# balazs-bamer/cuda-bezier-triangle-raytracer

Measured on AMD Instinct MI355X. Metric: Mrays/sec (primary+refracted) at 1/2/4/8 MI355X; % of HBM-read roofline, higher is better.
Workload: dtype f32; 1 GPU; cfg4: two stacked cfg2 lenses at x=10 and x=13, 4096x4096 rays; image=4096x4096, primaries_per_gpu=16777216, patches=6144, parallelism=64x64 image tiles round-robin over 1 rank(s), strong scaling, pipeline=fused, frames_in_flight=3, scan=BVH-culled (bit-identical to brute force), numerics=parity: bit-identical to the CPU oracle

## Files before the change

cuda-bezier-triangle-raytracer_amd/bzr_amd/__init__.py:

```python
from __future__ import annotations

import ctypes
import os
from contextlib import contextmanager
from pathlib import Path

import numpy as np

PKG_DIR = Path(__file__).resolve().parent.parent
LIB_PATH = Path(os.environ.get("BZR_LIBRARY", PKG_DIR / "lib" / "libbzr.so"))

OK = 0
HOST_PTRS, DEVICE_PTRS = 0, 1
MODE_PARITY, MODE_FAST = 0, 2
ACCEL_NONE = 4
PIPELINE_STAGED = 8
PIPELINE_FUSED = 16
RAYS_AOS = 32
WHAT_FOLLOW0, WHAT_FOLLOW1, WHAT_FOLLOW2, WHAT_NONE, WHAT_INTERSECT = 0, 1, 2, 3, 4
LIMIT_THIS, LIMIT_NONE = 0, 1
RR_NONE, RR_INSIDE, RR_OUTSIDE = 0, 1, 2
ENVELOPE_ELLIPSOID, ENVELOPE_TESTLENS = 0, 1
PATCH_WORDS = 66
KERNELS = ("k_traverse", "bucket", "k_newton", "k_follow", "k_finish", "k_overflow", "k_intersect_scan",
           "k_refract_scan", "k_chain_scan", "k_patch", "k_newton_lane", "k_trace")
COUNTERS = ("segments", "pairs", "follows", "overflow_rays", "lane_chunks", "node_visits", "leaf_fetches",
            "gate_tests", "newton_rounds", "rounds_odd", "runs_odd", "dirty_rows")
HIT_FIELDS = 13

_P = ctypes.c_void_p
_U32 = ctypes.c_uint32
_I32 = ctypes.c_int32
_F = ctypes.c_float

_SIGS = {
    "bzr_abi_version": [],
    "bzr_last_error": [],
    "bzr_device_count": [ctypes.POINTER(_I32)],
    "bzr_ctx_create": [_I32, ctypes.POINTER(_P)],
    "bzr_ctx_destroy": [_P],
    "bzr_ctx_set_stream": [_P, _P],
    "bzr_ctx_use_own_stream": [_P],
# ... 616 lines not shown
```

cuda-bezier-triangle-raytracer_amd/csrc/device/patch_math.hpp:

```cpp
#pragma once
#include <hip/hip_runtime.h>
#include <cfloat>
#include <cstdint>

namespace bzr_dev {

struct f3 {
  float x, y, z;
};
__device__ __forceinline__ f3 mk(float x, float y, float z) { return f3{x, y, z}; }
namespace rec {
constexpr int kUnder = 0;
constexpr int kDivider = 4;
constexpr int kNeigh = 16;
constexpr int kCp = 19;
constexpr int kMinv = 49;
constexpr int kHin = 58;
constexpr int kHout = 59;
constexpr int kDirA = 60;
constexpr int kDirB = 63;
constexpr int kWords = 66;
}

struct Patch {
// ... 153 lines not shown
__device__ __forceinline__ f3 unit_or_self(f3 a, float z) {
  if (!(z > 0.0f)) return a;
  float r = __builtin_amdgcn_rsqf(z);
  return mk(a.x * r, a.y * r, a.z * r);
}
__device__ __forceinline__ void div_heights(float hin, float hout, float ic, float &din, float &dout) {
  din = div_rn(hin, ic);
  dout = div_rn(hout, ic);
}
#include "patch_math_body.inc"
#pragma clang fp contract(off)
}

using namespace exact;

template <bool kGated = false, bool kFast = false, typename P>
__device__ __forceinline__ Hit patch_intersect(const P &p, f3 s, f3 d, bool limitNone) {
  Hit h;
  h.t = 0.0f;
  h.point = mk(0.0f, 0.0f, 0.0f);
  h.cs = 0.0f;
  h.bary = h.point;
  h.normal = h.point;
  h.what = kNone;
  f3 ip;
  float ic, it;
  bool valid = plane_ray(p.n(), p.c(), s, d, ip, ic, it);
  (void)valid;
#if BZR_PASS_FLAT
  if (!kGated) {
    const f3 b0 = matvec(p, ip);
    const bool in = (b0.x >= 0.0f) & (b0.x <= 1.0f) & (b0.y >= 0.0f) & (b0.y <= 1.0f) & (b0.z >= 0.0f) & (b0.z <= 1.0f);
    const bool ok = valid & (fabsf(it) > -p.hin()) & (fabsf(it) > p.hout()) & (limitNone | in);
    Hit r;
    if constexpr (kFast) r = fast::newton_tail(p, s, d, ic, it);
    else r = newton_tail(p, s, d, ic, it);
    return ok ? r : h;
  }
#endif
  if (!kGated) {
    if (!(valid && fabsf(it) > -p.hin() && fabsf(it) > p.hout())) return h;
    f3 b0 = matvec(p, ip);
    if (!(limitNone || (b0.x >= 0.0f && b0.x <= 1.0f && b0.y >= 0.0f && b0.y <= 1.0f && b0.z >= 0.0f && b0.z <= 1.0f)))
      return h;
  }
  if constexpr (kFast) return fast::newton_tail(p, s, d, ic, it);
  else return newton_tail(p, s, d, ic, it);
}

}
```

cuda-bezier-triangle-raytracer_amd/csrc/device/patch_math_body.inc:

```
__device__ __forceinline__ f3 add(f3 a, f3 b) { return mk(a.x + b.x, a.y + b.y, a.z + b.z); }
__device__ __forceinline__ f3 sub(f3 a, f3 b) { return mk(a.x - b.x, a.y - b.y, a.z - b.z); }
__device__ __forceinline__ f3 scale(f3 a, float s) { return mk(a.x * s, a.y * s, a.z * s); }
__device__ __forceinline__ float dot(f3 a, f3 b) { return a.x * b.x + (a.y * b.y + a.z * b.z); }
__device__ __forceinline__ f3 cross(f3 a, f3 b) {
  return mk(a.y * b.z - a.z * b.y, a.z * b.x - a.x * b.z, a.x * b.y - a.y * b.x);
}
__device__ __forceinline__ f3 normalized(f3 a) {
  float z = dot(a, a);
  return unit_or_self(a, z);
}

template <typename P>
__device__ __forceinline__ f3 matvec(const P &p, f3 v) {
  return mk(p.m(0) * v.x + (p.m(3) * v.y + p.m(6) * v.z), p.m(1) * v.x + (p.m(4) * v.y + p.m(7) * v.z),
            p.m(2) * v.x + (p.m(5) * v.y + p.m(8) * v.z));
}

__device__ __forceinline__ bool plane_ray(f3 n, float c, f3 start, f3 dir, f3 &point, float &cs, float &t) {
  cs = dot(dir, n);
  if (fabsf(cs) >= 0.00001f) {
    t = div_rn(c - dot(n, start), cs);
    point = add(start, scale(dir, t));
    return t > 0.0f;
  }
// ... 30 lines not shown
  f3 k0 = mk(BZR_K0(x), BZR_K0(y), BZR_K0(z));
  f3 k1 = mk(BZR_K1(x), BZR_K1(y), BZR_K1(z));
  f3 k2 = mk(BZR_K2(x), BZR_K2(y), BZR_K2(z));
#undef BZR_K0
#undef BZR_K1
#undef BZR_K2
#undef c
  const f3 da = p.da(), db = p.db();
  f3 ca = mk((da.x * k0.x + da.y * k1.x) + da.z * k2.x, (da.x * k0.y + da.y * k1.y) + da.z * k2.y,
             (da.x * k0.z + da.y * k1.z) + da.z * k2.z);
  f3 cb = mk((db.x * k0.x + db.y * k1.x) + db.z * k2.x, (db.x * k0.y + db.y * k1.y) + db.z * k2.y,
             (db.x * k0.z + db.y * k1.z) + db.z * k2.z);
  return normalized(cross(ca, cb));
}

template <typename P>
__device__ __forceinline__ Hit newton_tail(const P &p, f3 s, f3 d, float ic, float it) {
  Hit h;
  h.t = 0.0f;
  h.point = mk(0.0f, 0.0f, 0.0f);
  h.cs = 0.0f;
  h.bary = h.point;
  h.normal = h.point;
  h.what = kNone;
  float din, dout;
  div_heights(p.hin(), p.hout(), ic, din, dout);
  float closer = it + (ic > 0.0f ? din : dout);
  float further = it + (ic > 0.0f ? dout : din);
  f3 por = add(s, scale(d, closer));
  f3 b = matvec(p, plane_project(p.n(), p.c(), por));
  f3 q = interpolate(p, b);
  float diffc = fabsf(plane_distance(p.n(), p.c(), por)) - fabsf(plane_distance(p.n(), p.c(), q));
  por = add(s, scale(d, further));
  b = matvec(p, plane_project(p.n(), p.c(), por));
  q = interpolate(p, b);
  float difff = fabsf(plane_distance(p.n(), p.c(), por)) - fabsf(plane_distance(p.n(), p.c(), q));
  float den = diffc - difff;
  float middle = fabsf(den) < 0.000001f ? div_rn(closer + further, 2.0f)
                                        : div_rn(diffc * further - difff * closer, den);
  f3 pdir = p.n();
#if BZR_NEWTON_UNROLL
#pragma unroll
#endif
  for (int i = 0; i < BZR_NEWTON_ITERS; ++i) {
    h.t = middle;
    por = add(s, scale(d, middle));
    f3 pp;
    float pc, pt;
    plane_ray(p.n(), p.c(), por, pdir, pp, pc, pt);
    h.bary = matvec(p, pp);
    h.normal = surface_normal(p, h.bary);
    h.point = interpolate(p, h.bary);
    pdir = normalized(sub(h.point, pp));
    middle = div_rn(dot(sub(h.point, s), h.normal), dot(d, h.normal));
#ifdef BZR_NEWTON_PROBE
    BZR_NEWTON_PROBE(i, middle, pdir);
#endif
  }
  f3 rel = sub(h.point, s);
  f3 perp = sub(rel, scale(d, dot(rel, d)));
  if (sqrt_above_hundredth(dot(perp, perp)) || h.t < (further - closer) * 1.0f) {
    h.what = kNone;
    return h;
  }
  uint32_t out = plane_distance(p.dn(0), p.dc(0), h.point) < 0.0f ? 1u : 0u;
  out |= plane_distance(p.dn(1), p.dc(1), h.point) < 0.0f ? 2u : 0u;
  out |= plane_distance(p.dn(2), p.dc(2), h.point) < 0.0f ? 4u : 0u;
  if (out == 1u) h.what = 0u;
  else if (out == 2u) h.what = 1u;
  else if (out == 4u) h.what = 2u;
  else {
    h.what = kIntersect;
    h.cs = dot(d, h.normal);
  }
  return h;
}
```

cuda-bezier-triangle-raytracer_amd/csrc/device/trace.hip:

```cpp
#include <hip/hip_runtime.h>
#include <hipcub/hipcub.hpp>

#include <algorithm>
#include <climits>
#include <cstdlib>
#include <functional>

#include <cstdio>
#include <cstring>
#include <new>
#include <type_traits>
#include <string>
#include <vector>

#include "../host/bvh.hpp"
#include "bzr.h"
#include "ctx.hpp"
#include "patch_math.hpp"
#include "emitter.hpp"

using namespace bzr_dev;

namespace {
thread_local std::string t_error;
// ... 167 lines not shown
  hits[(size_t)9 * n + i] = h.normal.y;
  hits[(size_t)10 * n + i] = h.normal.z;
  reinterpret_cast<uint32_t *>(hits)[(size_t)11 * n + i] = h.what;
  reinterpret_cast<uint32_t *>(hits)[(size_t)12 * n + i] = patch;
}

__device__ __forceinline__ Hit no_hit() {
  Hit h;
  h.t = FLT_MAX;
  h.what = kNone;
  h.point = h.bary = h.normal = mk(0.0f, 0.0f, 0.0f);
  h.cs = 0.0f;
  return h;
}

__device__ __forceinline__ bool planar_gate(float4 q0, float4 q1, float4 q2, float4 q3, f3 s, f3 d) {
#if BZR_GATE_FLAT
  const f3 n = mk(q0.x, q0.y, q0.z);
  const float cs = dot(d, n);
  const float t = div_rn(q0.w - dot(n, s), cs);
  const f3 ip = add(s, scale(d, t));
  const bool valid = (fabsf(cs) >= 0.00001f) & (t > 0.0f) & (fabsf(t) > -q1.x) & (fabsf(t) > q1.y);
  const float b0 = q1.z * ip.x + (q1.w * ip.y + q2.x * ip.z);
  const float b1 = q2.y * ip.x + (q2.z * ip.y + q2.w * ip.z);
  const float b2 = q3.x * ip.x + (q3.y * ip.y + q3.z * ip.z);
  return valid & (b0 >= 0.0f) & (b0 <= 1.0f) & (b1 >= 0.0f) & (b1 <= 1.0f) & (b2 >= 0.0f) & (b2 <= 1.0f);
#else
  f3 n = mk(q0.x, q0.y, q0.z);
  f3 ip;
  float ic, it;
  bool valid = plane_ray(n, q0.w, s, d, ip, ic, it);
  if (!(valid && fabsf(it) > -q1.x && fabsf(it) > q1.y)) return false;
  float b0 = q1.z * ip.x + (q1.w * ip.y + q2.x * ip.z);
  float b1 = q2.y * ip.x + (q2.z * ip.y + q2.w * ip.z);
  float b2 = q3.x * ip.x + (q3.y * ip.y + q3.z * ip.z);
  return b0 >= 0.0f && b0 <= 1.0f && b1 >= 0.0f && b1 <= 1.0f && b2 >= 0.0f && b2 <= 1.0f;
#endif
}

template <bool kFast = false>
__device__ __forceinline__ Hit evaluate_patch(const MeshView &m, uint32_t b, f3 s, f3 d, uint32_t &src) {
  uint32_t idx = b;
  bool limitNone = false;
  Hit h;
  for (int pass = 0; pass < 2; ++pass) {
    Patch p = load_patch(m.full + (size_t)rec::kWords * idx);
    h = patch_intersect<false, kFast>(p, s, d, limitNone);
    if (pass == 0 && h.what <= kFollow2) {
      idx = __float_as_uint(m.full[(size_t)rec::kWords * idx + rec::kNeigh + h.what]);
      limitNone = true;
      continue;
    }
// ... 209 lines not shown
  write_slot(slot, n, ray, j, h, src);
#if !BZR_RECORD_RET
  atomicMin(key, k);
#endif
}

__device__ __forceinline__ float4 leaf_q(const u32x16 &r, int g) {
  return make_float4(__uint_as_float(r[4 * g]), __uint_as_float(r[4 * g + 1]), __uint_as_float(r[4 * g + 2]),
                     g == 3 ? 0.0f : __uint_as_float(r[4 * g + 3]));
}

constexpr uint32_t kAlwaysQuads = 8;
typedef uint32_t u32x8 __attribute__((ext_vector_type(8)));
typedef __attribute__((address_space(4))) const u32x8 cu32x8;

__device__ __forceinline__ bool always_gate_rec(const u32x16 &r, const u32x8 &wq, bool act, f3 s, f3 d, uint32_t &patch) {
  patch = r[15];
  const float4 q0 = leaf_q(r, 0);
  const f3 n = mk(q0.x, q0.y, q0.z);
  const float cs = dot(d, n), num = q0.w - dot(n, s);
  bool keep = act & (fabsf(cs) >= 0.00001f) & (((num > 0.0f) & (cs > 0.0f)) | ((num < 0.0f) & (cs < 0.0f)));
  keep |= act & ((num != num) | (cs != cs));
  if (!__any(keep)) return false;
  const float tt = num * __builtin_amdgcn_rcpf(cs);
  const f3 p = mk(__builtin_fmaf(d.x, tt, s.x), __builtin_fmaf(d.y, tt, s.y), __builtin_fmaf(d.z, tt, s.z));
  const float pm = fmaxf(fmaxf(fabsf(p.x), fabsf(p.y)), fabsf(p.z)), sm = fmaxf(fmaxf(fabsf(s.x), fabsf(s.y)), fabsf(s.z));
  const float w = __builtin_fmaf(__uint_as_float(wq[0]), p.x, __builtin_fmaf(__uint_as_float(wq[1]), p.y, __uint_as_float(wq[2]) * p.z));
  const float slack = __builtin_fmaf(__uint_as_float(wq[5]), pm, __uint_as_float(wq[6]) * (sm + pm));
  keep &= !(w > __uint_as_float(wq[4]) + slack) & !(w < __uint_as_float(wq[3]) - slack);
  if (!__any(keep)) return false;
  return keep & planar_gate(q0, leaf_q(r, 1), leaf_q(r, 2), leaf_q(r, 3), s, d);
}
__device__ __forceinline__ bool always_gate(const float4 *always, uint32_t k, bool act, f3 s, f3 d, uint32_t &patch) {
  const u32x16 r = *((const cu32x16 *)(uintptr_t)(always + (size_t)kAlwaysQuads * k));
  const u32x8 wq = *((const cu32x8 *)(uintptr_t)(always + (size_t)kAlwaysQuads * k + 4));
  return always_gate_rec(r, wq, act, s, d, patch);
}

template <int kXor>
__device__ __forceinline__ float swz(float v) {
  return __int_as_float(__builtin_amdgcn_ds_swizzle(__float_as_int(v), 0x1F | (kXor << 10)));
}
__device__ __forceinline__ float halves(float v, bool mx) {
  const float a = __int_as_float(__builtin_amdgcn_readlane(__float_as_int(v), 0));
  const float b = __int_as_float(__builtin_amdgcn_readlane(__float_as_int(v), 32));
  return mx ? fmaxf(a, b) : fminf(a, b);
}
__device__ __forceinline__ float wave_minf(float v) {
  v = fminf(v, swz<1>(v));
  v = fminf(v, swz<2>(v));
  v = fminf(v, swz<4>(v));
// ... 927 lines not shown
  }
  if (lane == 63) wave_total[wv] = x;
  __syncthreads();
  unsigned long long before = 0;
  for (uint32_t k = 0; k < wv; ++k) before += wave_total[k];
  unsigned long long run = before + x - sum;
#pragma unroll
  for (uint32_t k = 0; k < kScanPer; ++k) {
    if (base + k < count) offs[base + k] = run;
    run += v[k];
  }
}

struct TraceCtr {
  uint32_t nodes = 0, leaves = 0, gate_tests = 0, rounds = 0, pairs = 0, follows = 0, segments = 0, ovf = 0;
  uint32_t rounds_odd = 0, runs_odd = 0;
};
#ifndef BZR_TRACE_PRIO
#define BZR_TRACE_PRIO 3
#endif
#ifndef BZR_TRACE_ENTRIES
#define BZR_TRACE_ENTRIES 16
#endif
#ifndef BZR_TRACE_SPEC
#define BZR_TRACE_SPEC 1
#endif
#ifndef BZR_TRACE_BUNDLE
#define BZR_TRACE_BUNDLE 1
#endif
#ifndef BZR_TRACE_PARK_HITS
#define BZR_TRACE_PARK_HITS 1
#endif
constexpr uint32_t kEntries = BZR_TRACE_ENTRIES;
static_assert(kEntries >= 4 && kEntries <= 64 && (kEntries & (kEntries - 1)) == 0, "kEntries");
template <int kMode>
struct TraceWords {
  static constexpr int kHit = kMode == kModeHits ? 12 : 7;
  static constexpr int kPark = !BZR_TRACE_SPEC ? 0 : (kMode != kModeHits ? 8 : (BZR_TRACE_PARK_HITS ? 11 : 0));
  static constexpr int kStackCap = (BZR_TRACE_BUNDLE && kMode != kModeHits) ? 2 * kStack : kStack;
};
template <int kMode>
struct TraceLds {
  uint32_t stack[TraceWords<kMode>::kStackCap];
  float hit[TraceWords<kMode>::kHit][64];
  unsigned long long emask[kEntries];
  float bundle[kBundleWords];
  uint32_t eid[kEntries];
#if BZR_TRACE_BUNDLE
  uint32_t pend[64];
#endif
  float park[TraceWords<kMode>::kPark ? TraceWords<kMode>::kPark : 1][64];
};

__device__ __forceinline__ uint32_t popc64(unsigned long long m) { return (uint32_t)__popcll(m); }
__device__ __forceinline__ unsigned long long uniform_u64(unsigned long long v) {
  const uint32_t hi = __builtin_amdgcn_readfirstlane((uint32_t)(v >> 32)), lo = __builtin_amdgcn_readfirstlane((uint32_t)v);
  return ((unsigned long long)hi << 32) | lo;
}
__device__ __forceinline__ bool lane_bit(unsigned long long m, uint32_t lane) { return ((m >> lane) & 1ull) != 0ull; }

template <int kMode>
__device__ __forceinline__ void consider(const Hit &h, uint32_t scan, uint32_t src, unsigned long long &best,
// ... 16 lines not shown
        L.hit[10][lane] = h.normal.z;
        L.hit[11][lane] = __uint_as_float(src);
      } else {
        L.hit[0][lane] = h.point.x;
        L.hit[1][lane] = h.point.y;
        L.hit[2][lane] = h.point.z;
        L.hit[3][lane] = h.cs;
        L.hit[4][lane] = h.normal.x;
        L.hit[5][lane] = h.normal.y;
        L.hit[6][lane] = h.normal.z;
      }
    }
  }
}

template <int kMode>
__device__ __forceinline__ Hit winner(TraceLds<kMode> &L, uint32_t lane, uint32_t &patch) {
  Hit h = no_hit();
  h.what = kIntersect;
  if constexpr (kMode == kModeHits) {
    h.t = L.hit[0][lane];
    h.point = mk(L.hit[1][lane], L.hit[2][lane], L.hit[3][lane]);
    h.cs = L.hit[4][lane];
    h.bary = mk(L.hit[5][lane], L.hit[6][lane], L.hit[7][lane]);
    h.normal = mk(L.hit[8][lane], L.hit[9][lane], L.hit[10][lane]);
    patch = __float_as_uint(L.hit[11][lane]);
  } else {
    h.point = mk(L.hit[0][lane], L.hit[1][lane], L.hit[2][lane]);
    h.cs = L.hit[3][lane];
    h.normal = mk(L.hit[4][lane], L.hit[5][lane], L.hit[6][lane]);
// ... 28 lines not shown
    h.point = mk(L.park[1][lane], L.park[2][lane], L.park[3][lane]);
    h.cs = L.park[4][lane];
    h.normal = mk(L.park[5][lane], L.park[6][lane], L.park[7][lane]);
    if constexpr (TraceWords<kMode>::kPark >= 11) h.bary = mk(L.park[8][lane], L.park[9][lane], L.park[10][lane]);
    h.what = kIntersect;
  }
  return h;
}

template <int kMode, bool kFast, bool kCount>
__device__ __forceinline__ void trace_segment(const MeshView &m, f3 s, f3 d, bool act, unsigned long long &best,
                                              TraceLds<kMode> &L, uint32_t lane, TraceCtr &ctr) {
  constexpr bool kPark = TraceWords<kMode>::kPark > 0;
  constexpr uint32_t kNo = 0xFFFFFFFFu;
  constexpr int kCap = TraceWords<kMode>::kStackCap;
  best = ~0ull;
  const float amax = fmaxf(fmaxf(fabsf(s.x), fabsf(s.y)), fabsf(s.z));
  bool ovf = false;
  if (act && !(amax <= m.s_max)) {
    ovf = true;
    act = false;
  }
  const bool near_tier = !__any(act && !(amax <= m.s_near));
  const bzr_host::Bvh4Node *nodes = near_tier ? m.nodes_near : m.nodes;
  const bzr_host::Bvh4ObbNode *obb = near_tier ? m.obb_near : m.obb;
  const float4 *leaf = near_tier ? m.leaf_near : m.leaf;
  const f3 inv = mk(safe_inv(d.x), safe_inv(d.y), safe_inv(d.z));
  const f3 sinv = mk(s.x * inv.x, s.y * inv.y, s.z * inv.z);
  int sp = 0;
  uint32_t next = (m.n > 0 && __any(act)) ? 0u : kNo;
// ... 18 lines not shown
    next = kNo;
    bwalk = true;
  }
#endif
  for (;;) {
    uint32_t ne = 0;
#if BZR_TRACE_PRIO
    __builtin_amdgcn_s_setprio(BZR_TRACE_PRIO);
#endif
#if BZR_TRACE_BUNDLE
    while (bwalk && ne < kEntries) {
      if (pi < npend) {
        const uint32_t slot = __builtin_amdgcn_readfirstlane(L.pend[pi]);
        ++pi;
        const u32x16 r = *((const cu32x16 *)(uintptr_t)leaf + slot);
        const bool pass = act & planar_gate(leaf_q(r, 0), leaf_q(r, 1), leaf_q(r, 2), leaf_q(r, 3), s, d);
        if (kCount) {
          ++ctr.leaves;
          ctr.gate_tests += popc64(__ballot(act));
        }
        const unsigned long long pm = __ballot(pass);
        if (pm) {
          if (lane == 0u) {
            L.eid[ne] = r[15];
            L.emask[ne] = pm;
          }
          ++ne;
        }
        continue;
      }
      if (sp == 0) break;
      pi = npend = 0;
      const uint32_t top = __builtin_amdgcn_readfirstlane(L.stack[sp - 1]);
      if (!narrow || (top & bzr_host::kObbFlag)) {
        --sp;
        if (kCount) ++ctr.nodes;
        bool hit[4];
        uint32_t ch[4];
        const f3 linv = mk(safe_inv(d.x), safe_inv(d.y), safe_inv(d.z));
        node_children(nodes, obb, top, act, s, d, mk(s.x * linv.x, s.y * linv.y, s.z * linv.z), linv, hit, ch);
// ... 29 lines not shown
      next = kNo;
      if (kCount) ++ctr.nodes;
      bool hit[4];
      uint32_t ch[4];
      node_children(nodes, obb, node, act, s, d, sinv, inv, hit, ch);
#pragma unroll
      for (int c = 0; c < 4; ++c) {
        const unsigned long long hm = __ballot(hit[c]);
        if (hm == 0ull) continue;
        if (ch[c] & bzr_host::kLeafFlag) {
          const u32x16 r = *((const cu32x16 *)(uintptr_t)leaf + (ch[c] & ~bzr_host::kLeafFlag));
          const float4 g0 = make_float4(__uint_as_float(r[0]), __uint_as_float(r[1]), __uint_as_float(r[2]), __uint_as_float(r[3]));
          const float4 g1 = make_float4(__uint_as_float(r[4]), __uint_as_float(r[5]), __uint_as_float(r[6]), __uint_as_float(r[7]));
          const float4 g2 = make_float4(__uint_as_float(r[8]), __uint_as_float(r[9]), __uint_as_float(r[10]), __uint_as_float(r[11]));
          const float4 g3 = make_float4(__uint_as_float(r[12]), __uint_as_float(r[13]), __uint_as_float(r[14]), 0.0f);
          const bool pass = hit[c] & planar_gate(g0, g1, g2, g3, s, d)
              ;
          if (kCount) {
            ++ctr.leaves;
            ctr.gate_tests += popc64(hm);
          }
          const unsigned long long pm = __ballot(pass);
          if (pm) {
            if (lane == 0u) {
              L.eid[ne] = r[15];
              L.emask[ne] = pm;
            }
            ++ne;
          }
        } else {
          if (next != kNo) {
            if (sp < kCap) L.stack[sp++] = next;
            else if (lane_bit(next_hm, lane)) ovf = true;
          }
          next = ch[c];
          next_hm = hm;
        }
      }
    }
#endif
    while (next == kNo && sp == 0 && ne < kEntries) {
      if (am == 0ull) {
        if (ab * 64u >= m.n_always) break;
        if (ab == 0u && !BZR_TRACE_BUNDLE) bundle_to_lds(act, s, d, L.bundle, lane);
        am = __ballot(always_bundle_keep(m.always, ab * 64u + lane, m.n_always, L.bundle));
        ++ab;
        continue;
      }
      const uint32_t k = (ab - 1u) * 64u + __builtin_ctzll(am);
      am &= am - 1ull;
      uint32_t b;
      const bool pass = always_gate(m.always, k, act, s, d, b);
      if (kCount) {
        ++ctr.leaves;
        ctr.gate_tests += popc64(__ballot(act));
      }
      const unsigned long long pm = __ballot(pass);
      if (pm) {
        if (lane == 0u) {
          L.eid[ne] = b;
          L.emask[ne] = pm;
        }
        ++ne;
      }
    }
    if (ne == 0u) {
#define BZR_SEG_END break;
      if (scan == kNo) {
        if (!__any(ovf)) BZR_SEG_END
        scan = 0;
        if (kCount) ctr.ovf += popc64(__ballot(ovf));
      }
      bool pass = false;
      for (; scan < m.n; ++scan) {
        const float4 *g = m.planar + 4u * scan;
        pass = ovf && planar_gate(g[0], g[1], g[2], g[3], s, d);
        if (__any(pass)) break;
      }
      if (scan >= m.n) BZR_SEG_END
#undef BZR_SEG_END
      const unsigned long long pm = __ballot(pass);
      if (lane == 0u) {
        L.eid[0] = scan;
        L.emask[0] = pm;
      }
      ne = 1;
      ++scan;
    }
#if BZR_TRACE_PRIO
    __builtin_amdgcn_s_setprio(0);
#endif
    for (uint32_t e = 0; e < ne; ++e) {
      const uint32_t b = __builtin_amdgcn_readfirstlane(L.eid[e]);
      const auto hp = uniform_patch(m.full, b);
      const bool run0 = lane_bit(uniform_u64(L.emask[e]), lane);
      const bool joined = join == b;
      const uint32_t sidx = joined ? join_src : b;
      if (joined) join = kNo;
      bool spec = false;
      if (kPark && e + 1u < ne) {
        unsigned long long sm = 0ull;
#pragma unroll
        for (uint32_t side = 0; side < 3u; ++side) {
          const uint32_t nb = __float_as_uint(hp.r[rec::kNeigh + side]);
          const unsigned long long later = __ballot(lane > e && lane < ne && L.eid[lane & (kEntries - 1u)] == nb);
          if (later) sm |= uniform_u64(L.emask[__builtin_ctzll(later)]);
        }
        spec = lane_bit(sm, lane) && !run0 && !joined && parked_nb == kNo;
      }
      if (kCount) {
        ++ctr.rounds;
        ctr.pairs += popc64(__ballot(run0));
        ctr.follows += popc64(__ballot(joined));
      }
      uint32_t what = kNone;
      if (run0 || joined || spec) {
        const Hit h = patch_intersect<false, kFast>(hp, s, d, joined || spec);
        if (spec) {
          park(h, L, lane);
          parked_nb = b;
        } else {
          consider(h, sidx, b, best, L, lane);
          if (!joined) what = h.what;
        }
      }
      for (uint32_t side = 0; side < 3u; ++side) {
        bool fl = run0 && what == side;
        if (!__any(fl)) continue;
        const uint32_t nb = __float_as_uint(hp.r[rec::kNeigh + side]);
        if (kPark) {
          const bool use = fl && parked_nb == nb;
          if (use) {
            consider(parked(L, lane), b, nb, best, L, lane);
            fl = false;
          }
          if (kCount) ctr.follows += popc64(__ballot(use));
          if (!__any(fl)) continue;
        }
        const unsigned long long later = __ballot(lane > e && lane < ne && L.eid[lane & (kEntries - 1u)] == nb);
        if (later) {
          const unsigned long long fm = uniform_u64(L.emask[__builtin_ctzll(later)]);
          if (fl && join == kNo && !lane_bit(fm, lane)) {
            join = nb;
            join_src = b;
            fl = false;
          }
        }
        if (!__any(fl)) continue;
        if (kCount) {
          ++ctr.rounds;
          ctr.follows += popc64(__ballot(fl));
        }
        const auto pa = uniform_patch(m.full, nb);
        if (fl) {
          const Hit h = patch_intersect<false, kFast>(pa, s, d, true);
          consider(h, b, nb, best, L, lane);
        }
      }
    }
  }
}

struct TraceJob {
  const float *rays;
  float *hits;
  float *out_rays;
  uint32_t *status;
  uint32_t *segments;
  const uint32_t *expected;
  const uint32_t *alive_in;
  uint32_t expected_all;
  uint32_t n;
// ... 142 lines not shown
  }
  if (job.cost && threadIdx.x == 0u) job.cost[tile] = sched_bin(__builtin_amdgcn_s_memtime() - t_start);
  if (job.wave_clock && lane == 0u) {
    const unsigned long long t_end = __builtin_amdgcn_s_memtime();
    if (job.wave_real) {
      const unsigned long long r_end = __builtin_amdgcn_s_memrealtime();
      job.wave_clock[4 * (i >> 6)] = t_start;
      job.wave_clock[4 * (i >> 6) + 1] = t_end - t_start;
      job.wave_clock[4 * (i >> 6) + 2] = r_start;
      job.wave_clock[4 * (i >> 6) + 3] = r_end - r_start;
    } else {
      job.wave_clock[2 * (i >> 6)] = t_start;
      job.wave_clock[2 * (i >> 6) + 1] = t_end - t_start;
    }
  }
  if (kCount && lane < 10u) {
    const uint32_t v[10] = {ctr.segments, ctr.pairs, ctr.follows, ctr.ovf, ctr.nodes, ctr.leaves, ctr.gate_tests,
                            ctr.rounds, ctr.rounds_odd, ctr.runs_odd};
    const uint32_t id[10] = {BZR_COUNTER_SEGMENTS, BZR_COUNTER_PAIRS, BZR_COUNTER_FOLLOWS, BZR_COUNTER_OVERFLOW_RAYS,
                             BZR_COUNTER_NODE_VISITS, BZR_COUNTER_LEAF_FETCHES, BZR_COUNTER_GATE_TESTS,
                             BZR_COUNTER_NEWTON_ROUNDS, BZR_COUNTER_ROUNDS_ODD, BZR_COUNTER_RUNS_ODD};
    uint32_t mine = 0, which = 0;
#pragma unroll
    for (uint32_t k = 0; k < 10u; ++k)
      if (lane == k) {
        mine = v[k];
        which = id[k];
      }
    const uint32_t rep = (blockIdx.x * kTraceWaves + (threadIdx.x >> 6)) % kCounterReplicas;
    if (mine) atomicAdd(&counters[(size_t)rep * BZR_COUNTER_COUNT + which], (unsigned long long)mine);
  }
}

__global__ __launch_bounds__(kBlock) void k_intersect_scan(MeshView m, const float *__restrict__ rays, uint32_t n,
                                                           float *__restrict__ hits) {
  uint32_t i = blockIdx.x * kBlock + threadIdx.x;
  if (i >= n) return;
  f3 s, d;
  load_ray(rays, n, i, s, d);
// ... 1401 lines not shown
```

cuda-bezier-triangle-raytracer_amd/csrc/host/capi_host.cpp:

```cpp
#include <cstring>
#include <new>
#include <string>

#include "bzr/bzr.hpp"

extern "C" void bzr_internal_set_error(const char *msg);

struct bzr_trimesh {
  Mesh mesh;
};

namespace {
template <typename F>
bzr_status guarded(F &&f) {
  try {
    f();
    return BZR_OK;
  } catch (char const *what) {
    bzr_internal_set_error(what);
    return BZR_ERR_PREPROCESS;
  } catch (std::bad_alloc const &) {
    bzr_internal_set_error("out of memory");
    return BZR_ERR_OUT_OF_MEMORY;
  } catch (std::out_of_range const &e) {
// ... 137 lines not shown
    if (bm.size()) std::memcpy(static_cast<void *>(out), &bm[0], sizeof(bzr_patch) * bm.size());
  });
}

bzr_status bzr_bezier_split_thick(const bzr_trimesh *m, bzr_trimesh *out) {
  if (!m || !out) return bad("null argument");
  return guarded([&] { out->mesh = BezierMesh(m->mesh).splitThickBezierTriangles(); });
}

bzr_status bzr_bezier_interpolate(const bzr_trimesh *m, int32_t divisor, bzr_trimesh *out) {
  if (!m || !out) return bad("null argument");
  if (divisor < 1) return bad("divisor must be >= 1");
  return guarded([&] { out->mesh = BezierMesh(m->mesh).interpolate(divisor); });
}

}
```

cuda-bezier-triangle-raytracer_amd/csrc/host/single_ray.cpp:

```cpp
#include <cfloat>
#include <cmath>
#include <cstdint>
#include <cstring>
#include <math.h>

#include "single_ray.hpp"

#define __device__
#define __forceinline__ inline
#define BZR_NEWTON_ITERS 4
#define BZR_NEWTON_UNROLL 0

namespace bzr_host {

struct f3 {
  float x, y, z;
};
inline f3 mk(float x, float y, float z) { return f3{x, y, z}; }
constexpr uint32_t kFollow2 = 2u, kNone = 3u, kIntersect = 4u;

struct Hit {
  float t;
  f3 point;
  float cs;
// ... 23 lines not shown
inline float sqrt_rn(float a) { return std::sqrt(a); }
inline bool sqrt_above_hundredth(float z) { return sqrt_rn(z) > 0.01f; }
inline f3 unit_or_self(f3 a, float z) {
  if (!(z > 0.0f)) return a;
  const float s = sqrt_rn(z);
  return mk(div_rn(a.x, s), div_rn(a.y, s), div_rn(a.z, s));
}
inline void div_heights(float hin, float hout, float ic, float &din, float &dout) {
  din = div_rn(hin, ic);
  dout = div_rn(hout, ic);
}
#include "../device/patch_math_body.inc"
}
using namespace exact;

Hit patch_intersect(const PatchView &p, f3 s, f3 d, bool limitNone) {
  Hit h;
  h.t = 0.0f;
  h.point = mk(0.0f, 0.0f, 0.0f);
  h.cs = 0.0f;
  h.bary = h.point;
  h.normal = h.point;
  h.what = kNone;
  f3 ip;
  float ic, it;
  const bool valid = plane_ray(p.n(), p.c(), s, d, ip, ic, it);
  if (!(valid && fabsf(it) > -p.hin() && fabsf(it) > p.hout())) return h;
  const f3 b0 = matvec(p, ip);
  if (!(limitNone || (b0.x >= 0.0f && b0.x <= 1.0f && b0.y >= 0.0f && b0.y <= 1.0f && b0.z >= 0.0f && b0.z <= 1.0f)))
    return h;
  return newton_tail(p, s, d, ic, it);
}

Hit no_hit() {
  Hit h;
  h.t = FLT_MAX;
  h.what = kNone;
  h.point = h.bary = h.normal = mk(0.0f, 0.0f, 0.0f);
  h.cs = 0.0f;
  return h;
}

Hit mesh_intersect(const float *records, std::size_t n, f3 s, f3 d, uint32_t &patch) {
  Hit best = no_hit();
  patch = 0xFFFFFFFFu;
  for (std::size_t b = 0; b < n; ++b) {
// ... 26 lines not shown
    if (s2 < 0.99f) {
      if (s2 > 1e-12f) {
        const float sgn = st == BZR_RR_INSIDE ? 1.0f : -1.0f;
        const f3 nn = scale(h.normal, sgn);
        const float c1 = fabsf(h.cs);
        const float c2 = sqrt_rn(1.0f - s2);
        o_d = normalized(add(scale(d, eta), scale(nn, eta * c1 - c2)));
      }
    } else {
      st = BZR_RR_NONE;
    }
  }
  return st == expected ? st : uint32_t(BZR_RR_NONE);
}

f3 v3(Vector const &v) { return mk(v(0), v(1), v(2)); }
Vector vec(f3 v) { return Vector(v.x, v.y, v.z); }

BezierIntersection to_reference(const Hit &h) {
  BezierIntersection b;
  b.mIntersection.mDistance = h.t;
  b.mIntersection.mPoint = vec(h.point);
  b.mIntersection.mCosIncidence = h.cs;
  b.mIntersection.mValid = h.what == kIntersect;
  b.mBarycentric = vec(h.bary);
  b.mNormal = vec(h.normal);
  b.mWhat = static_cast<BezierIntersection::What>(h.what);
  return b;
}

// ... 42 lines not shown
```

cuda-bezier-triangle-raytracer_amd/csrc/host/single_ray.hpp:

```cpp
#pragma once
#include <cstddef>
#include <cstdint>
#include <utility>

#include "bzr/bzr.hpp"

namespace bzr {
namespace host {
BezierIntersection patchIntersect(BezierTriangle const &patch, Ray const &ray, bool limitNone);
BezierIntersection meshIntersect(BezierTriangle const *patches, std::size_t n, Ray const &ray, uint32_t *patch);
std::pair<Ray, RefractionResult> lensRefract(BezierTriangle const *patches, std::size_t n, float ri, Ray const &ray,
                                             RefractionResult expected);
}
}
```

include/bzr.h:

```cpp
#ifndef BZR_H
#define BZR_H

#include <stddef.h>
#include <stdint.h>

#ifdef __cplusplus
extern "C" {
#endif

#define BZR_ABI_VERSION 2

typedef int32_t bzr_status;
enum {
  BZR_OK = 0,
  BZR_ERR_INVALID_ARGUMENT = 1,
  BZR_ERR_HIP = 2,
  BZR_ERR_OUT_OF_MEMORY = 3,
  BZR_ERR_PREPROCESS = 4,
  BZR_ERR_NO_DEVICE = 5,
  BZR_ERR_CAPACITY = 6
};

enum {
  BZR_HOST_PTRS = 0u,
// ... 54 lines not shown
bzr_status bzr_ctx_timing(bzr_ctx *ctx, int32_t enable);
bzr_status bzr_ctx_timing_report(bzr_ctx *ctx, float ms[BZR_KERNEL_COUNT], uint32_t calls[BZR_KERNEL_COUNT]);

enum {
  BZR_COUNTER_SEGMENTS = 0,
  BZR_COUNTER_PAIRS = 1,
  BZR_COUNTER_FOLLOWS = 2,
  BZR_COUNTER_OVERFLOW_RAYS = 3,
  BZR_COUNTER_LANE_CHUNKS = 4,
  BZR_COUNTER_NODE_VISITS = 5,
  BZR_COUNTER_LEAF_FETCHES = 6,
  BZR_COUNTER_GATE_TESTS = 7,
  BZR_COUNTER_NEWTON_ROUNDS = 8,
  BZR_COUNTER_ROUNDS_ODD = 9,
  BZR_COUNTER_RUNS_ODD = 10,
  BZR_COUNTER_DIRTY_ROWS = 11,
  BZR_COUNTER_COUNT = 12
};
bzr_status bzr_ctx_counters(bzr_ctx *ctx, int32_t enable);
bzr_status bzr_ctx_counters_report(bzr_ctx *ctx, uint64_t counts[BZR_COUNTER_COUNT]);

bzr_status bzr_mesh_create(bzr_ctx *ctx, const void *patches, uint32_t n, uint32_t stride, bzr_mesh **out);
bzr_status bzr_mesh_destroy(bzr_mesh *mesh);
bzr_status bzr_mesh_size(const bzr_mesh *mesh, uint32_t *n);

bzr_status bzr_intersect(bzr_ctx *ctx, const bzr_mesh *mesh, const float *rays_soa, uint32_t n,
                         float *hits_soa, uint32_t flags);
typedef struct bzr_hit_record {
  uint32_t valid;
  float    point[3];
  float    cos_incidence;
// ... 89 lines not shown
```

include/bzr_debug.h:

```cpp
#ifndef BZR_DEBUG_H
#define BZR_DEBUG_H
#include <stdint.h>
#ifdef __cplusplus
extern "C" {
#endif
int32_t bzr_debug_gate_boxes(const void *patches, uint32_t n, uint32_t stride, float *boxes, float *s_max);
int32_t bzr_debug_gate_boxes_tier(const void *patches, uint32_t n, uint32_t stride, int32_t tier, float *boxes,
                                  float *s_max);
int32_t bzr_debug_always_list(const void *patches, uint32_t n, uint32_t stride, int32_t tier, uint32_t *out,
                              uint32_t *count);
int32_t bzr_debug_always_wedges(const void *patches, uint32_t n, uint32_t stride, int32_t tier, float *out);
int32_t bzr_debug_gate_obbs(const void *patches, uint32_t n, uint32_t stride, int32_t tier, float *out);
int32_t bzr_debug_bounding_sphere(const void *patches, uint32_t n, uint32_t stride, float out[4]);
int32_t bzr_debug_traverse(const void *patches, uint32_t n, uint32_t stride, const float *rays, uint32_t nr,
                           uint8_t *hits, uint64_t stats[4]);
int32_t bzr_debug_traverse_bundle(const void *patches, uint32_t n, uint32_t stride, const float *rays, uint32_t nr,
                                  float max_spread, uint64_t stats[12]);
int32_t bzr_debug_unit(void *ctx, const float *a, uint32_t n, float *out);
int32_t bzr_debug_div_heights(void *ctx, const float *a, uint32_t n, float *out);
int32_t bzr_debug_fast_unit(void *ctx, const float *a, uint32_t n, float *out);
int32_t bzr_debug_chunk_plan(uint64_t free_bytes, uint64_t n, uint32_t *cap, uint32_t *chunk);
int32_t bzr_debug_chunk_cap(void *ctx, uint32_t rays, uint32_t *effective);
int32_t bzr_debug_wave_clock(void *ctx, unsigned long long *clock, uint32_t waves);
int32_t bzr_debug_wave_clock_rate(void *ctx, unsigned long long *clock, uint32_t waves);
#ifdef __cplusplus
}
#endif
#endif
```

Before: 11470 Mrays/s.

## Sort gate-passing entries by plane distance and skip final Newton normal when beaten

Peels the last Newton iteration so the surface-normal evaluation becomes conditional. A wave-wide vote skips it when no lane's candidate t can beat the current best hit. Gate-passing leaf entries are also ranked by their planar-gate t, so nearer patches are intersected first and the best hit tightens sooner. This adds a readlane rank loop, LDS reshuffles and an extra key array per entry, and the skipped normals are zeroed, which relies on those hits being discarded.

```diff
diff --git a/cuda-bezier-triangle-raytracer_amd/bzr_amd/__init__.py b/cuda-bezier-triangle-raytracer_amd/bzr_amd/__init__.py
--- a/cuda-bezier-triangle-raytracer_amd/bzr_amd/__init__.py
+++ b/cuda-bezier-triangle-raytracer_amd/bzr_amd/__init__.py
@@ -25,7 +25,7 @@
 KERNELS = ("k_traverse", "bucket", "k_newton", "k_follow", "k_finish", "k_overflow", "k_intersect_scan",
            "k_refract_scan", "k_chain_scan", "k_patch", "k_newton_lane", "k_trace")
 COUNTERS = ("segments", "pairs", "follows", "overflow_rays", "lane_chunks", "node_visits", "leaf_fetches",
-            "gate_tests", "newton_rounds", "rounds_odd", "runs_odd", "dirty_rows")
+            "gate_tests", "newton_rounds", "rounds_odd", "runs_odd", "short_passes")
 HIT_FIELDS = 13
 
 _P = ctypes.c_void_p
diff --git a/cuda-bezier-triangle-raytracer_amd/csrc/device/patch_math.hpp b/cuda-bezier-triangle-raytracer_amd/csrc/device/patch_math.hpp
--- a/cuda-bezier-triangle-raytracer_amd/csrc/device/patch_math.hpp
+++ b/cuda-bezier-triangle-raytracer_amd/csrc/device/patch_math.hpp
@@ -191,8 +191,8 @@
 
 using namespace exact;
 
-template <bool kGated = false, bool kFast = false, typename P>
-__device__ __forceinline__ Hit patch_intersect(const P &p, f3 s, f3 d, bool limitNone) {
+template <bool kGated = false, bool kFast = false, typename P, typename Need = NormalAlways>
+__device__ __forceinline__ Hit patch_intersect(const P &p, f3 s, f3 d, bool limitNone, Need need = Need()) {
   Hit h;
   h.t = 0.0f;
   h.point = mk(0.0f, 0.0f, 0.0f);
@@ -210,8 +210,8 @@
     const bool in = (b0.x >= 0.0f) & (b0.x <= 1.0f) & (b0.y >= 0.0f) & (b0.y <= 1.0f) & (b0.z >= 0.0f) & (b0.z <= 1.0f);
     const bool ok = valid & (fabsf(it) > -p.hin()) & (fabsf(it) > p.hout()) & (limitNone | in);
     Hit r;
-    if constexpr (kFast) r = fast::newton_tail(p, s, d, ic, it);
-    else r = newton_tail(p, s, d, ic, it);
+    if constexpr (kFast) r = fast::newton_tail(p, s, d, ic, it, need);
+    else r = newton_tail(p, s, d, ic, it, need);
     return ok ? r : h;
   }
 #endif
@@ -221,8 +221,8 @@
     if (!(limitNone || (b0.x >= 0.0f && b0.x <= 1.0f && b0.y >= 0.0f && b0.y <= 1.0f && b0.z >= 0.0f && b0.z <= 1.0f)))
       return h;
   }
-  if constexpr (kFast) return fast::newton_tail(p, s, d, ic, it);
-  else return newton_tail(p, s, d, ic, it);
-}
-
-}
+  if constexpr (kFast) return fast::newton_tail(p, s, d, ic, it, need);
+  else return newton_tail(p, s, d, ic, it, need);
+}
+
+}
diff --git a/cuda-bezier-triangle-raytracer_amd/csrc/device/patch_math_body.inc b/cuda-bezier-triangle-raytracer_amd/csrc/device/patch_math_body.inc
--- a/cuda-bezier-triangle-raytracer_amd/csrc/device/patch_math_body.inc
+++ b/cuda-bezier-triangle-raytracer_amd/csrc/device/patch_math_body.inc
@@ -68,8 +68,11 @@
   return normalized(cross(ca, cb));
 }
 
-template <typename P>
-__device__ __forceinline__ Hit newton_tail(const P &p, f3 s, f3 d, float ic, float it) {
+struct NormalAlways {
+  __device__ __forceinline__ bool operator()(float) const { return true; }
+};
+template <typename P, typename Need = NormalAlways>
+__device__ __forceinline__ Hit newton_tail(const P &p, f3 s, f3 d, float ic, float it, Need need = Need()) {
   Hit h;
   h.t = 0.0f;
   h.point = mk(0.0f, 0.0f, 0.0f);
@@ -96,7 +99,7 @@
 #if BZR_NEWTON_UNROLL
 #pragma unroll
 #endif
-  for (int i = 0; i < BZR_NEWTON_ITERS; ++i) {
+  for (int i = 0; i + 1 < BZR_NEWTON_ITERS; ++i) {
     h.t = middle;
     por = add(s, scale(d, middle));
     f3 pp;
@@ -111,21 +114,33 @@
     BZR_NEWTON_PROBE(i, middle, pdir);
 #endif
   }
+  h.t = middle;
+  por = add(s, scale(d, middle));
+  f3 pp;
+  float pc, pt;
+  plane_ray(p.n(), p.c(), por, pdir, pp, pc, pt);
+  h.bary = matvec(p, pp);
+  h.point = interpolate(p, h.bary);
   f3 rel = sub(h.point, s);
   f3 perp = sub(rel, scale(d, dot(rel, d)));
-  if (sqrt_above_hundredth(dot(perp, perp)) || h.t < (further - closer) * 1.0f) {
-    h.what = kNone;
-    return h;
+  uint32_t what = kNone;
+  if (!(sqrt_above_hundredth(dot(perp, perp)) || h.t < (further - closer) * 1.0f)) {
+    uint32_t out = plane_distance(p.dn(0), p.dc(0), h.point) < 0.0f ? 1u : 0u;
+    out |= plane_distance(p.dn(1), p.dc(1), h.point) < 0.0f ? 2u : 0u;
+    out |= plane_distance(p.dn(2), p.dc(2), h.point) < 0.0f ? 4u : 0u;
+    what = out == 1u ? 0u : (out == 2u ? 1u : (out == 4u ? 2u : kIntersect));
   }
-  uint32_t out = plane_distance(p.dn(0), p.dc(0), h.point) < 0.0f ? 1u : 0u;
-  out |= plane_distance(p.dn(1), p.dc(1), h.point) < 0.0f ? 2u : 0u;
-  out |= plane_distance(p.dn(2), p.dc(2), h.point) < 0.0f ? 4u : 0u;
-  if (out == 1u) h.what = 0u;
-  else if (out == 2u) h.what = 1u;
-  else if (out == 4u) h.what = 2u;
-  else {
-    h.what = kIntersect;
-    h.cs = dot(d, h.normal);
+  h.what = what;
+  if (need(h.t)) {
+    h.normal = surface_normal(p, h.bary);
+    if (what == kIntersect) h.cs = dot(d, h.normal);
+#ifdef BZR_NEWTON_PROBE
+    pdir = normalized(sub(h.point, pp));
+    middle = div_rn(dot(sub(h.point, s), h.normal), dot(d, h.normal));
+    BZR_NEWTON_PROBE(BZR_NEWTON_ITERS - 1, middle, pdir);
+#endif
+  } else {
+    h.normal = mk(0.0f, 0.0f, 0.0f);
   }
   return h;
 }
diff --git a/cuda-bezier-triangle-raytracer_amd/csrc/device/trace.hip b/cuda-bezier-triangle-raytracer_amd/csrc/device/trace.hip
--- a/cuda-bezier-triangle-raytracer_amd/csrc/device/trace.hip
+++ b/cuda-bezier-triangle-raytracer_amd/csrc/device/trace.hip
@@ -205,12 +205,13 @@
   return h;
 }
 
-__device__ __forceinline__ bool planar_gate(float4 q0, float4 q1, float4 q2, float4 q3, f3 s, f3 d) {
+__device__ __forceinline__ bool planar_gate(float4 q0, float4 q1, float4 q2, float4 q3, f3 s, f3 d, float &gt) {
 #if BZR_GATE_FLAT
   const f3 n = mk(q0.x, q0.y, q0.z);
   const float cs = dot(d, n);
   const float t = div_rn(q0.w - dot(n, s), cs);
   const f3 ip = add(s, scale(d, t));
+  gt = t;
   const bool valid = (fabsf(cs) >= 0.00001f) & (t > 0.0f) & (fabsf(t) > -q1.x) & (fabsf(t) > q1.y);
   const float b0 = q1.z * ip.x + (q1.w * ip.y + q2.x * ip.z);
   const float b1 = q2.y * ip.x + (q2.z * ip.y + q2.w * ip.z);
@@ -221,12 +222,17 @@
   f3 ip;
   float ic, it;
   bool valid = plane_ray(n, q0.w, s, d, ip, ic, it);
+  gt = it;
   if (!(valid && fabsf(it) > -q1.x && fabsf(it) > q1.y)) return false;
   float b0 = q1.z * ip.x + (q1.w * ip.y + q2.x * ip.z);
   float b1 = q2.y * ip.x + (q2.z * ip.y + q2.w * ip.z);
   float b2 = q3.x * ip.x + (q3.y * ip.y + q3.z * ip.z);
   return b0 >= 0.0f && b0 <= 1.0f && b1 >= 0.0f && b1 <= 1.0f && b2 >= 0.0f && b2 <= 1.0f;
 #endif
+}
+__device__ __forceinline__ bool planar_gate(float4 q0, float4 q1, float4 q2, float4 q3, f3 s, f3 d) {
+  float gt;
+  return planar_gate(q0, q1, q2, q3, s, d, gt);
 }
 
 template <bool kFast = false>
@@ -466,8 +472,10 @@
 typedef uint32_t u32x8 __attribute__((ext_vector_type(8)));
 typedef __attribute__((address_space(4))) const u32x8 cu32x8;
 
-__device__ __forceinline__ bool always_gate_rec(const u32x16 &r, const u32x8 &wq, bool act, f3 s, f3 d, uint32_t &patch) {
+__device__ __forceinline__ bool always_gate_rec(const u32x16 &r, const u32x8 &wq, bool act, f3 s, f3 d, uint32_t &patch,
+                                                float &gt) {
   patch = r[15];
+  gt = 0.0f;
   const float4 q0 = leaf_q(r, 0);
   const f3 n = mk(q0.x, q0.y, q0.z);
   const float cs = dot(d, n), num = q0.w - dot(n, s);
@@ -481,12 +489,21 @@
   const float slack = __builtin_fmaf(__uint_as_float(wq[5]), pm, __uint_as_float(wq[6]) * (sm + pm));
   keep &= !(w > __uint_as_float(wq[4]) + slack) & !(w < __uint_as_float(wq[3]) - slack);
   if (!__any(keep)) return false;
-  return keep & planar_gate(q0, leaf_q(r, 1), leaf_q(r, 2), leaf_q(r, 3), s, d);
-}
-__device__ __forceinline__ bool always_gate(const float4 *always, uint32_t k, bool act, f3 s, f3 d, uint32_t &patch) {
+  return keep & planar_gate(q0, leaf_q(r, 1), leaf_q(r, 2), leaf_q(r, 3), s, d, gt);
+}
+__device__ __forceinline__ bool always_gate_rec(const u32x16 &r, const u32x8 &wq, bool act, f3 s, f3 d, uint32_t &patch) {
+  float gt;
+  return always_gate_rec(r, wq, act, s, d, patch, gt);
+}
+__device__ __forceinline__ bool always_gate(const float4 *always, uint32_t k, bool act, f3 s, f3 d, uint32_t &patch,
+                                            float &gt) {
   const u32x16 r = *((const cu32x16 *)(uintptr_t)(always + (size_t)kAlwaysQuads * k));
   const u32x8 wq = *((const cu32x8 *)(uintptr_t)(always + (size_t)kAlwaysQuads * k + 4));
-  return always_gate_rec(r, wq, act, s, d, patch);
+  return always_gate_rec(r, wq, act, s, d, patch, gt);
+}
+__device__ __forceinline__ bool always_gate(const float4 *always, uint32_t k, bool act, f3 s, f3 d, uint32_t &patch) {
+  float gt;
+  return always_gate(always, k, act, s, d, patch, gt);
 }
 
 template <int kXor>
@@ -1444,6 +1461,7 @@
 
 struct TraceCtr {
   uint32_t nodes = 0, leaves = 0, gate_tests = 0, rounds = 0, pairs = 0, follows = 0, segments = 0, ovf = 0;
+  uint32_t shorts = 0;
   uint32_t rounds_odd = 0, runs_odd = 0;
 };
 #ifndef BZR_TRACE_PRIO
@@ -1461,6 +1479,10 @@
 #ifndef BZR_TRACE_PARK_HITS
 #define BZR_TRACE_PARK_HITS 1
 #endif
+#ifndef BZR_TRACE_SHORT
+#define BZR_TRACE_SHORT 1
+#endif
+static_assert(BZR_TRACE_SHORT >= 0 && BZR_TRACE_SHORT <= 2, "BZR_TRACE_SHORT: 0, 1 or 2");
 constexpr uint32_t kEntries = BZR_TRACE_ENTRIES;
 static_assert(kEntries >= 4 && kEntries <= 64 && (kEntries & (kEntries - 1)) == 0, "kEntries");
 template <int kMode>
@@ -1476,6 +1498,9 @@
   unsigned long long emask[kEntries];
   float bundle[kBundleWords];
   uint32_t eid[kEntries];
+#if BZR_TRACE_SHORT == 1
+  uint32_t ekey[kEntries];
+#endif
 #if BZR_TRACE_BUNDLE
   uint32_t pend[64];
 #endif
@@ -1522,6 +1547,28 @@
   }
 }
 
+struct PassVote {
+  unsigned long long best;
+  uint32_t scan;
+  bool spec;
+  bool *skipped;
+  __device__ __forceinline__ bool operator()(float t) const {
+#if BZR_TRACE_SHORT
+    const bool may = spec || (t < FLT_MAX && (((unsigned long long)t_order(t) << 32) | scan) < best);
+    const bool any = __any(may);
+    *skipped = !any;
+    return any;
+#else
+    (void)t;
+    return true;
+#endif
+  }
+};
+
+__device__ __forceinline__ uint32_t entry_key(float gt, unsigned long long pm) {
+  return t_order(__int_as_float(__builtin_amdgcn_readlane(__float_as_int(gt), (int)__builtin_ctzll(pm))));
+}
+
 template <int kMode>
 __device__ __forceinline__ Hit winner(TraceLds<kMode> &L, uint32_t lane, uint32_t &patch) {
   Hit h = no_hit();
@@ -1580,6 +1627,7 @@
   constexpr bool kPark = TraceWords<kMode>::kPark > 0;
   constexpr uint32_t kNo = 0xFFFFFFFFu;
   constexpr int kCap = TraceWords<kMode>::kStackCap;
+  constexpr bool kOrder = BZR_TRACE_SHORT == 1;
   best = ~0ull;
   const float amax = fmaxf(fmaxf(fabsf(s.x), fabsf(s.y)), fabsf(s.z));
   bool ovf = false;
@@ -1628,16 +1676,22 @@
         const uint32_t slot = __builtin_amdgcn_readfirstlane(L.pend[pi]);
         ++pi;
         const u32x16 r = *((const cu32x16 *)(uintptr_t)leaf + slot);
-        const bool pass = act & planar_gate(leaf_q(r, 0), leaf_q(r, 1), leaf_q(r, 2), leaf_q(r, 3), s, d);
+        float gt;
+        const bool pass = act & planar_gate(leaf_q(r, 0), leaf_q(r, 1), leaf_q(r, 2), leaf_q(r, 3), s, d, gt);
         if (kCount) {
           ++ctr.leaves;
           ctr.gate_tests += popc64(__ballot(act));
         }
         const unsigned long long pm = __ballot(pass);
         if (pm) {
+          const uint32_t key = kOrder ? entry_key(gt, pm) : 0u;
+          (void)key;
           if (lane == 0u) {
             L.eid[ne] = r[15];
             L.emask[ne] = pm;
+#if BZR_TRACE_SHORT == 1
+            L.ekey[ne] = key;
+#endif
           }
           ++ne;
         }
@@ -1697,17 +1751,22 @@
           const float4 g1 = make_float4(__uint_as_float(r[4]), __uint_as_float(r[5]), __uint_as_float(r[6]), __uint_as_float(r[7]));
           const float4 g2 = make_float4(__uint_as_float(r[8]), __uint_as_float(r[9]), __uint_as_float(r[10]), __uint_as_float(r[11]));
           const float4 g3 = make_float4(__uint_as_float(r[12]), __uint_as_float(r[13]), __uint_as_float(r[14]), 0.0f);
-          const bool pass = hit[c] & planar_gate(g0, g1, g2, g3, s, d)
-              ;
+          float gt;
+          const bool pass = hit[c] & planar_gate(g0, g1, g2, g3, s, d, gt);
           if (kCount) {
             ++ctr.leaves;
             ctr.gate_tests += popc64(hm);
           }
           const unsigned long long pm = __ballot(pass);
           if (pm) {
+            const uint32_t key = kOrder ? entry_key(gt, pm) : 0u;
+            (void)key;
             if (lane == 0u) {
               L.eid[ne] = r[15];
               L.emask[ne] = pm;
+#if BZR_TRACE_SHORT == 1
+              L.ekey[ne] = key;
+#endif
             }
             ++ne;
           }
@@ -1733,16 +1792,22 @@
       const uint32_t k = (ab - 1u) * 64u + __builtin_ctzll(am);
       am &= am - 1ull;
       uint32_t b;
-      const bool pass = always_gate(m.always, k, act, s, d, b);
+      float gt;
+      const bool pass = always_gate(m.always, k, act, s, d, b, gt);
       if (kCount) {
         ++ctr.leaves;
         ctr.gate_tests += popc64(__ballot(act));
       }
       const unsigned long long pm = __ballot(pass);
       if (pm) {
+        const uint32_t key = kOrder ? entry_key(gt, pm) : 0u;
+        (void)key;
         if (lane == 0u) {
           L.eid[ne] = b;
           L.emask[ne] = pm;
+#if BZR_TRACE_SHORT == 1
+          L.ekey[ne] = key;
+#endif
         }
         ++ne;
       }
@@ -1773,6 +1838,27 @@
 #if BZR_TRACE_PRIO
     __builtin_amdgcn_s_setprio(0);
 #endif
+    if (kOrder && ne >= 2u) {
+      const uint32_t slot = lane & (kEntries - 1u);
+#if BZR_TRACE_SHORT == 1
+      const uint32_t ekey = L.ekey[slot];
+#else
+      const uint32_t ekey = 0u;
+#endif
+      uint32_t rank = 0;
+      for (uint32_t j = 0; j < ne; ++j) {
+        const uint32_t kj = (uint32_t)__builtin_amdgcn_readlane((int)ekey, (int)j);
+        rank += (kj < ekey || (kj == ekey && j < lane)) ? 1u : 0u;
+      }
+      const uint32_t id = L.eid[slot];
+      const unsigned long long em = L.emask[slot];
+      __builtin_amdgcn_wave_barrier();
+      if (lane < ne) {
+        L.eid[rank] = id;
+        L.emask[rank] = em;
+      }
+      __builtin_amdgcn_wave_barrier();
+    }
     for (uint32_t e = 0; e < ne; ++e) {
       const uint32_t b = __builtin_amdgcn_readfirstlane(L.eid[e]);
       const auto hp = uniform_patch(m.full, b);
@@ -1797,8 +1883,9 @@
         ctr.follows += popc64(__ballot(joined));
       }
       uint32_t what = kNone;
+      bool skipped = false;
       if (run0 || joined || spec) {
-        const Hit h = patch_intersect<false, kFast>(hp, s, d, joined || spec);
+        const Hit h = patch_intersect<false, kFast>(hp, s, d, joined || spec, PassVote{best, sidx, spec, &skipped});
         if (spec) {
           park(h, L, lane);
           parked_nb = b;
@@ -1807,6 +1894,7 @@
           if (!joined) what = h.what;
         }
       }
+      if (kCount && __any(skipped)) ++ctr.shorts;
       for (uint32_t side = 0; side < 3u; ++side) {
         bool fl = run0 && what == side;
         if (!__any(fl)) continue;
@@ -1835,10 +1923,12 @@
           ctr.follows += popc64(__ballot(fl));
         }
         const auto pa = uniform_patch(m.full, nb);
+        skipped = false;
         if (fl) {
-          const Hit h = patch_intersect<false, kFast>(pa, s, d, true);
+          const Hit h = patch_intersect<false, kFast>(pa, s, d, true, PassVote{best, b, false, &skipped});
           consider(h, b, nb, best, L, lane);
         }
+        if (kCount && __any(skipped)) ++ctr.shorts;
       }
     }
   }
@@ -2011,15 +2101,16 @@
       job.wave_clock[2 * (i >> 6) + 1] = t_end - t_start;
     }
   }
-  if (kCount && lane < 10u) {
-    const uint32_t v[10] = {ctr.segments, ctr.pairs, ctr.follows, ctr.ovf, ctr.nodes, ctr.leaves, ctr.gate_tests,
-                            ctr.rounds, ctr.rounds_odd, ctr.runs_odd};
-    const uint32_t id[10] = {BZR_COUNTER_SEGMENTS, BZR_COUNTER_PAIRS, BZR_COUNTER_FOLLOWS, BZR_COUNTER_OVERFLOW_RAYS,
+  if (kCount && lane < 11u) {
+    const uint32_t v[11] = {ctr.segments, ctr.pairs, ctr.follows, ctr.ovf, ctr.nodes, ctr.leaves, ctr.gate_tests,
+                            ctr.rounds, ctr.rounds_odd, ctr.runs_odd, ctr.shorts};
+    const uint32_t id[11] = {BZR_COUNTER_SEGMENTS, BZR_COUNTER_PAIRS, BZR_COUNTER_FOLLOWS, BZR_COUNTER_OVERFLOW_RAYS,
                              BZR_COUNTER_NODE_VISITS, BZR_COUNTER_LEAF_FETCHES, BZR_COUNTER_GATE_TESTS,
-                             BZR_COUNTER_NEWTON_ROUNDS, BZR_COUNTER_ROUNDS_ODD, BZR_COUNTER_RUNS_ODD};
+                             BZR_COUNTER_NEWTON_ROUNDS, BZR_COUNTER_ROUNDS_ODD, BZR_COUNTER_RUNS_ODD,
+                             BZR_COUNTER_SHORT_PASSES};
     uint32_t mine = 0, which = 0;
 #pragma unroll
-    for (uint32_t k = 0; k < 10u; ++k)
+    for (uint32_t k = 0; k < 11u; ++k)
       if (lane == k) {
         mine = v[k];
         which = id[k];
diff --git a/cuda-bezier-triangle-raytracer_amd/csrc/host/capi_host.cpp b/cuda-bezier-triangle-raytracer_amd/csrc/host/capi_host.cpp
--- a/cuda-bezier-triangle-raytracer_amd/csrc/host/capi_host.cpp
+++ b/cuda-bezier-triangle-raytracer_amd/csrc/host/capi_host.cpp
@@ -3,6 +3,7 @@
 #include <string>
 
 #include "bzr/bzr.hpp"
+#include "single_ray.hpp"
 
 extern "C" void bzr_internal_set_error(const char *msg);
 
@@ -175,4 +176,23 @@
   return guarded([&] { out->mesh = BezierMesh(m->mesh).interpolate(divisor); });
 }
 
+int32_t bzr_debug_newton_short(const void *patches, uint32_t n, uint32_t stride, const uint32_t *patch,
+                               const float *rays, const uint8_t *limit, uint32_t m, float *full, float *skipped) {
+  if ((!patches && n) || ((!patch || !rays || !limit || !full || !skipped) && m)) return bad("null argument");
+  if (stride < sizeof(bzr_patch) || stride % 4u) return bad("stride");
+  for (uint32_t i = 0; i < m; ++i)
+    if (patch[i] >= n) return bad("patch index out of range");
+  for (uint32_t i = 0; i < m; ++i) {
+    const float *rec = reinterpret_cast<const float *>(static_cast<const char *>(patches) + (std::size_t)stride * patch[i]);
+    const float ray[6] = {rays[i],
+                          rays[(std::size_t)m + i],
+                          rays[(std::size_t)2 * m + i],
+                          rays[(std::size_t)3 * m + i],
+                          rays[(std::size_t)4 * m + i],
+                          rays[(std::size_t)5 * m + i]};
+    bzr_host::newton_short_pair(rec, ray, limit[i] != 0, full + (std::size_t)12 * i, skipped + (std::size_t)12 * i);
+  }
+  return BZR_OK;
 }
+
+}
diff --git a/cuda-bezier-triangle-raytracer_amd/csrc/host/single_ray.cpp b/cuda-bezier-triangle-raytracer_amd/csrc/host/single_ray.cpp
--- a/cuda-bezier-triangle-raytracer_amd/csrc/host/single_ray.cpp
+++ b/cuda-bezier-triangle-raytracer_amd/csrc/host/single_ray.cpp
@@ -61,7 +61,8 @@
 }
 using namespace exact;
 
-Hit patch_intersect(const PatchView &p, f3 s, f3 d, bool limitNone) {
+template <typename Need = NormalAlways>
+Hit patch_intersect(const PatchView &p, f3 s, f3 d, bool limitNone, Need need = Need()) {
   Hit h;
   h.t = 0.0f;
   h.point = mk(0.0f, 0.0f, 0.0f);
@@ -76,7 +77,7 @@
   const f3 b0 = matvec(p, ip);
   if (!(limitNone || (b0.x >= 0.0f && b0.x <= 1.0f && b0.y >= 0.0f && b0.y <= 1.0f && b0.z >= 0.0f && b0.z <= 1.0f)))
     return h;
-  return newton_tail(p, s, d, ic, it);
+  return newton_tail(p, s, d, ic, it, need);
 }
 
 Hit no_hit() {
@@ -133,6 +134,22 @@
   return st == expected ? st : uint32_t(BZR_RR_NONE);
 }
 
+struct NormalNever {
+  bool operator()(float) const { return false; }
+};
+void put_hit(const Hit &h, float out[12]) {
+  const float w[11] = {h.t,      h.point.x, h.point.y,  h.point.z,  h.cs,      h.bary.x,
+                       h.bary.y, h.bary.z,  h.normal.x, h.normal.y, h.normal.z};
+  std::memcpy(out, w, sizeof w);
+  std::memcpy(out + 11, &h.what, 4);
+}
+void newton_short_pair(const float *record, const float ray[6], bool limitNone, float full[12], float skipped[12]) {
+  const PatchView p{record};
+  const f3 s = mk(ray[0], ray[1], ray[2]), d = mk(ray[3], ray[4], ray[5]);
+  put_hit(patch_intersect(p, s, d, limitNone), full);
+  put_hit(patch_intersect(p, s, d, limitNone, NormalNever()), skipped);
+}
+
 f3 v3(Vector const &v) { return mk(v(0), v(1), v(2)); }
 Vector vec(f3 v) { return Vector(v.x, v.y, v.z); }
 
diff --git a/cuda-bezier-triangle-raytracer_amd/csrc/host/single_ray.hpp b/cuda-bezier-triangle-raytracer_amd/csrc/host/single_ray.hpp
--- a/cuda-bezier-triangle-raytracer_amd/csrc/host/single_ray.hpp
+++ b/cuda-bezier-triangle-raytracer_amd/csrc/host/single_ray.hpp
@@ -4,6 +4,10 @@
 #include <utility>
 
 #include "bzr/bzr.hpp"
+
+namespace bzr_host {
+void newton_short_pair(const float *record, const float ray[6], bool limitNone, float full[12], float skipped[12]);
+}
 
 namespace bzr {
 namespace host {
diff --git a/include/bzr.h b/include/bzr.h
--- a/include/bzr.h
+++ b/include/bzr.h
@@ -92,7 +92,7 @@
   BZR_COUNTER_NEWTON_ROUNDS = 8,
   BZR_COUNTER_ROUNDS_ODD = 9,
   BZR_COUNTER_RUNS_ODD = 10,
-  BZR_COUNTER_DIRTY_ROWS = 11,
+  BZR_COUNTER_SHORT_PASSES = 11,
   BZR_COUNTER_COUNT = 12
 };
 bzr_status bzr_ctx_counters(bzr_ctx *ctx, int32_t enable);
diff --git a/include/bzr_debug.h b/include/bzr_debug.h
--- a/include/bzr_debug.h
+++ b/include/bzr_debug.h
@@ -23,6 +23,8 @@
 int32_t bzr_debug_chunk_cap(void *ctx, uint32_t rays, uint32_t *effective);
 int32_t bzr_debug_wave_clock(void *ctx, unsigned long long *clock, uint32_t waves);
 int32_t bzr_debug_wave_clock_rate(void *ctx, unsigned long long *clock, uint32_t waves);
+int32_t bzr_debug_newton_short(const void *patches, uint32_t n, uint32_t stride, const uint32_t *patch,
+                               const float *rays, const uint8_t *limit, uint32_t m, float *full, float *skipped);
 #ifdef __cplusplus
 }
 #endif
```

Result: faster. 11670 Mrays/s (median of 6 runs) (+1.7%).
